# owl-project/owlExaBrick

Measured on AMD Instinct MI355X. Metric: frames/sec at 2048^2 DVR, exajet-like, MI355X, higher is better.
Workload: dtype f32; 1 GPU; c4_exajet (seed 0xe7a0003 procedural AMR, scale 1.0): 640512000 cells / 1251000 bricks / 13349488 regions, 2048x2048 DVR, dt 0.5, alpha ramp, gradient shading on, space skipping on, frameID 0; tiling=16x16 tiles interleaved over 1 GPU(s)

## Files before the change

### owlexabrick_amd/csrc/exa_kernels.hip

```cpp
#include "exa_device.h"
#include <cfloat>

#if EXA_BASIS_FORM == 0 && EXA_EMPTY_CELLS
#define EXA_FORM_NS form0e
#elif EXA_BASIS_FORM == 0
#define EXA_FORM_NS form0
#elif EXA_BASIS_FORM == 1 && EXA_EMPTY_CELLS
#error "empty cells are a per-corner property: the per-axis association (EXA_BASIS_FORM 1) does not apply"
#elif EXA_BASIS_FORM == 1
#define EXA_FORM_NS form1
#else
#error "EXA_BASIS_FORM is 0 (source order) or 1 (per-axis association with fused multiply-adds)"
#endif
#define EXA_F1 (EXA_BASIS_FORM == 1)
#ifndef EXA_TU_ROPE
#define EXA_TU_ROPE 0
#endif
#ifndef EXA_TU_SAMPLE
#define EXA_TU_SAMPLE 0
#endif
#ifndef EXA_TU_STREAM
#define EXA_TU_STREAM 0
#endif
namespace exa {
namespace EXA_FORM_NS {

struct V3 { float x, y, z; };
__device__ __forceinline__ V3 mk(float x, float y, float z) { V3 r; r.x = x; r.y = y; r.z = z; return r; }
__device__ __forceinline__ V3 mk(const float *p) { return mk(p[0], p[1], p[2]); }
__device__ __forceinline__ V3 operator+(V3 a, V3 b) { return mk(a.x + b.x, a.y + b.y, a.z + b.z); }
__device__ __forceinline__ V3 operator-(V3 a, V3 b) { return mk(a.x - b.x, a.y - b.y, a.z - b.z); }
__device__ __forceinline__ V3 operator*(float s, V3 a) { return mk(s * a.x, s * a.y, s * a.z); }
__device__ __forceinline__ V3 operator-(V3 a) { return mk(-a.x, -a.y, -a.z); }
__device__ __forceinline__ float dot(V3 a, V3 b) { return a.x * b.x + a.y * b.y + a.z * b.z; }
__device__ __forceinline__ float dotF(V3 a, V3 b) { return EXA_F1 ? __builtin_fmaf(a.z, b.z, __builtin_fmaf(a.y, b.y, a.x * b.x)) : dot(a, b); }
__device__ __forceinline__ V3 gradOf(float sumW, float sumWV, V3 sumD, V3 sumDC)
{
  return EXA_F1 ? mk(__builtin_fmaf(sumW, sumD.x, -(sumWV * sumDC.x)), __builtin_fmaf(sumW, sumD.y, -(sumWV * sumDC.y)),
                     __builtin_fmaf(sumW, sumD.z, -(sumWV * sumDC.z)))
                : mk(sumW * sumD.x - sumWV * sumDC.x, sumW * sumD.y - sumWV * sumDC.y, sumW * sumD.z - sumWV * sumDC.z);
}
__device__ __forceinline__ V3 rayAt(V3 org, float t, V3 dir)
{ return EXA_F1 ? mk(__builtin_fmaf(t, dir.x, org.x), __builtin_fmaf(t, dir.y, org.y), __builtin_fmaf(t, dir.z, org.z)) : org + t * dir; }
__device__ __forceinline__ float length(V3 a) { return sqrtf(dot(a, a)); }
__device__ __forceinline__ V3 normalize(V3 a) { return (1.f / sqrtf(dot(a, a))) * a; }
__device__ __forceinline__ V3 cross(V3 a, V3 b)
{ return mk(a.y * b.z - a.z * b.y, a.z * b.x - a.x * b.z, a.x * b.y - a.y * b.x); }

__device__ __forceinline__ V3 xfmPoint(const ExaHipFrameState &fs, V3 p)
{ return p.x * mk(fs.xfm_vx) + (p.y * mk(fs.xfm_vy) + (p.z * mk(fs.xfm_vz) + mk(fs.xfm_p))); }
__device__ __forceinline__ V3 xfmVector(const ExaHipFrameState &fs, V3 v)
{ return v.x * mk(fs.xfm_vx) + (v.y * mk(fs.xfm_vy) + v.z * mk(fs.xfm_vz)); }

struct Lcg {
  uint32_t state;
  __device__ __forceinline__ void init(uint32_t v0, uint32_t v1)
  {
    uint32_t s0 = 0;
#pragma unroll
    for (int n = 0; n < 16; n++) {
      s0 += 0x9e3779b9u;
      v0 += ((v1 << 4) + 0xa341316cu) ^ (v1 + s0) ^ ((v1 >> 5) + 0xc8013ea4u);
      v1 += ((v0 << 4) + 0xad90777du) ^ (v0 + s0) ^ ((v0 >> 5) + 0x7e95761eu);
    }
    state = v0;
  }
  __device__ __forceinline__ float next()
  {
    state = 1664525u * state + 1013904223u;
    return float(state & 0x00FFFFFFu) / float(0x01000000);
  }
};

template <bool FAST> __device__ __forceinline__ float fdiv(float a, float b) { return FAST ? a * __builtin_amdgcn_rcpf(b) : a / b; }
template <bool FAST> __device__ __forceinline__ float fdivExact(float a, float b, float y )
{
  if (!FAST) return a / b;
  const float q = __builtin_amdgcn_fmed3f(a * y, -3.402823466e+38f, 3.402823466e+38f);
  return __builtin_fmaf(__builtin_fmaf(-q, b, a), y, q);
}
template <bool FAST> __device__ __forceinline__ float fdivExact(float a, float b) { return fdivExact<FAST>(a, b, FAST ? __builtin_amdgcn_rcpf(b) : 0.f); }
template <bool FAST> __device__ __forceinline__ float fsqrt(float a) { return FAST ? __builtin_amdgcn_sqrtf(a) : sqrtf(a); }

struct Ray { V3 org, dir; float tmin, tmax; };
// ... 143 lines not shown
    if (ha && hb) {
      const bool aFirst = a0 <= b0;
      stack[sp * 256] = aFirst ? cc.y : cc.x;
      sp++;
      node = aFirst ? cc.x : cc.y;
    } else if (ha) {
      node = cc.x;
    } else if (hb) {
      node = cc.y;
    } else {
      if (sp == 0) break;
      sp--;
      node = stack[sp * 256];
    }
  }
  return best;
}

struct Basis { float sumWV, sumW; V3 sumD, sumDC; };

template <bool DERIV, int STATS>
__device__ __forceinline__ void addBasisFunctions(Ctx<STATS> &C, Basis &B, const int4 b0, const int4 b1,
                                                  const float *__restrict__ field, V3 pos)
{
  const int sx = b0.w, sy = b1.x, sz = b1.y;
  const float invCw = __int_as_float((127 - b1.z) << 23);
  const float lpx = (pos.x - float(b0.x)) * invCw - 0.5f;
  const float lpy = (pos.y - float(b0.y)) * invCw - 0.5f;
  const float lpz = (pos.z - float(b0.z)) * invCw - 0.5f;
  const int lx = max(-1, int(floorf(lpx))), ly = max(-1, int(floorf(lpy))), lz = max(-1, int(floorf(lpz)));
  const int hx = lx + 1, hy = ly + 1, hz = lz + 1;
  const float fx = lpx - float(lx), fy = lpy - float(ly), fz = lpz - float(lz);
  const float nx = 1.f - fx, ny = 1.f - fy, nz = 1.f - fz;
  const bool vlx = lx >= 0 && lx < sx, vhx = hx < sx;
  const bool vly = ly >= 0 && ly < sy, vhy = hy < sy;
  const bool vlz = lz >= 0 && lz < sz, vhz = hz < sz;
  const int cxl = min(max(lx, 0), sx - 1), cxh = min(hx, sx - 1);
  const int cyl = min(max(ly, 0), sy - 1), cyh = min(hy, sy - 1);
  const int czl = min(max(lz, 0), sz - 1), czh = min(hz, sz - 1);
  const uint32_t base = (uint32_t)b1.w;
  const uint32_t rowLL = base + (uint32_t)(cyl * sx + czl * sx * sy);
  const uint32_t rowHL = base + (uint32_t)(cyh * sx + czl * sx * sy);
  const uint32_t rowLH = base + (uint32_t)(cyl * sx + czh * sx * sy);
  const uint32_t rowHH = base + (uint32_t)(cyh * sx + czh * sx * sy);
  const float s000 = field[rowLL + cxl], s100 = field[rowLL + cxh];
  const float s010 = field[rowHL + cxl], s110 = field[rowHL + cxh];
  const float s001 = field[rowLH + cxl], s101 = field[rowLH + cxh];
  const float s011 = field[rowHH + cxl], s111 = field[rowHH + cxh];
  C.count(ST_BRICK_VISITS);
#define EXA_CORNER(VALID, S, WZ, WY, WX, SGX, SGY, SGZ)                                     \
  {                                                                                          \
     \
    const bool v_ = (VALID) && (!EXA_EMPTY_CELLS || (S) != EXA_EMPTY_CELL_POISON_VALUE);     \
    if (STATS == 1 && (VALID)) C.st[ST_CORNER_LOADS]++;                                      \
    const float w_ = (WZ) * (WY) * (WX);                                                     \
    if (DERIV) {                                                                             \
      const float dx_ = (WZ) * (WY) * (SGX 1.f);                                             \
      const float dy_ = (WZ) * (WX) * (SGY 1.f);                                             \
      const float dz_ = (WY) * (WX) * (SGZ 1.f);                                             \
      B.sumDC.x = v_ ? B.sumDC.x + dx_ : B.sumDC.x;                                          \
      B.sumDC.y = v_ ? B.sumDC.y + dy_ : B.sumDC.y;                                          \
      B.sumDC.z = v_ ? B.sumDC.z + dz_ : B.sumDC.z;                                          \
      B.sumD.x = v_ ? B.sumD.x + dx_ * (S) : B.sumD.x;                                       \
      B.sumD.y = v_ ? B.sumD.y + dy_ * (S) : B.sumD.y;                                       \
      B.sumD.z = v_ ? B.sumD.z + dz_ * (S) : B.sumD.z;                                       \
    }                                                                                        \
    B.sumW = v_ ? B.sumW + w_ : B.sumW;                                                      \
    B.sumWV = v_ ? B.sumWV + w_ * (S) : B.sumWV;                                             \
  }
  EXA_CORNER(vlz && vly && vlx, s000, nz, ny, nx, -, -, -)
  EXA_CORNER(vlz && vly && vhx, s100, nz, ny, fx, +, -, -)
  EXA_CORNER(vlz && vhy && vlx, s010, nz, fy, nx, -, +, -)
  EXA_CORNER(vlz && vhy && vhx, s110, nz, fy, fx, +, +, -)
  EXA_CORNER(vhz && vly && vlx, s001, fz, ny, nx, -, -, +)
  EXA_CORNER(vhz && vly && vhx, s101, fz, ny, fx, +, -, +)
  EXA_CORNER(vhz && vhy && vlx, s011, fz, fy, nx, -, +, +)
  EXA_CORNER(vhz && vhy && vhx, s111, fz, fy, fx, +, +, +)
#undef EXA_CORNER
}

struct __attribute__((packed, aligned(4))) Pair { float a, b; };
__device__ __forceinline__ Pair loadPair(const float *__restrict__ p) { return *reinterpret_cast<const Pair *>(p); }

template <bool DERIV, int STATS, bool SMALL, bool VOXEL = false, bool CUBE = false>
__device__ __forceinline__ void addBasisFast(Ctx<STATS> &C, Basis &B, const int4 b0, const int4 b1,
                                             const float *__restrict__ field, V3 pos, const int cubeLog2 = 0)
{
  static_assert(!CUBE || SMALL, "cube records: the 32-bit address form only");
  const int sx = CUBE ? (1 << cubeLog2) : b1.x, sy = CUBE ? sx : b1.y, sz = CUBE ? sx : b1.z;
  const uint32_t begin = CUBE ? ((uint32_t)b0.w >> 9) << (3 * cubeLog2) : (uint32_t)b1.w;
  const float invCw = __int_as_float(CUBE ? (int)((uint32_t)b0.w << 23) : b0.w);
  const float lpx = EXA_F1 ? __builtin_fmaf(pos.x - __int_as_float(b0.x), invCw, -0.5f) : (pos.x - __int_as_float(b0.x)) * invCw - 0.5f;
  const float lpy = EXA_F1 ? __builtin_fmaf(pos.y - __int_as_float(b0.y), invCw, -0.5f) : (pos.y - __int_as_float(b0.y)) * invCw - 0.5f;
  const float lpz = EXA_F1 ? __builtin_fmaf(pos.z - __int_as_float(b0.z), invCw, -0.5f) : (pos.z - __int_as_float(b0.z)) * invCw - 0.5f;
  const float flx = fmaxf(floorf(lpx), -1.f), fly = fmaxf(floorf(lpy), -1.f), flz = fmaxf(floorf(lpz), -1.f);
  const int lx = int(flx), ly = int(fly), lz = int(flz);
  const int hx = lx + 1, hy = ly + 1, hz = lz + 1;
  const float fx = lpx - flx, fy = lpy - fly, fz = lpz - flz;
  const bool vlx = (uint32_t)lx < (uint32_t)sx, vhx = hx < sx;
  const bool vly = (uint32_t)ly < (uint32_t)sy, vhy = hy < sy;
  const bool vlz = (uint32_t)lz < (uint32_t)sz, vhz = hz < sz;
  auto med3 = [](int a, int c) {
    int r;
    if (CUBE) asm("v_med3_i32 %0, %1, 0, %2" : "=v"(r) : "v"(a), "s"(c));
    else asm("v_med3_i32 %0, %1, 0, %2" : "=v"(r) : "v"(a), "v"(c));
    return r;
  };
  const int cxl = med3(lx, sx - 1), cxh = min(hx, sx - 1);
  const int cyl = med3(ly, sy - 1), cyh = min(hy, sy - 1);
  const int czl = med3(lz, sz - 1), czh = min(hz, sz - 1);
  const int bx = med3(lx, CUBE ? sx - 2 : max(sx - 2, 0));
  float s000, s100, s010, s110, s001, s101, s011, s111;
  {
    uint32_t rowLL, rowHL, rowLH, rowHH;
    if (CUBE) {
      const uint32_t at = begin + (uint32_t)bx;
      const uint32_t zl = ((uint32_t)czl << (2 * cubeLog2)) + at, zh = ((uint32_t)czh << (2 * cubeLog2)) + at;
      rowLL = ((uint32_t)cyl << cubeLog2) + zl; rowHL = ((uint32_t)cyh << cubeLog2) + zl;
      rowLH = ((uint32_t)cyl << cubeLog2) + zh; rowHH = ((uint32_t)cyh << cubeLog2) + zh;
    } else if (SMALL) {
      const uint32_t sxy = __umul24((uint32_t)sx, (uint32_t)sy);
      const uint32_t zl = __umul24((uint32_t)czl, sxy) + (begin + (uint32_t)bx);
      const uint32_t zh = __umul24((uint32_t)czh, sxy) + (begin + (uint32_t)bx);
      const uint32_t yl = __umul24((uint32_t)cyl, (uint32_t)sx), yh = __umul24((uint32_t)cyh, (uint32_t)sx);
      rowLL = zl + yl; rowHL = zl + yh; rowLH = zh + yl; rowHH = zh + yh;
    } else {
      const uint32_t sxy = (uint32_t)(sx * sy);
      const uint32_t zl = begin + (uint32_t)czl * sxy + (uint32_t)bx, zh = begin + (uint32_t)czh * sxy + (uint32_t)bx;
      const uint32_t yl = (uint32_t)(cyl * sx), yh = (uint32_t)(cyh * sx);
      rowLL = zl + yl; rowHL = zl + yh; rowLH = zh + yl; rowHH = zh + yh;
    }
    const bool lFirst = cxl == bx, hFirst = cxh == bx;
    Pair pLL, pHL, pLH, pHH;
    if (SMALL) {
      const char *base = reinterpret_cast<const char *>(field);
      pLL = *reinterpret_cast<const Pair *>(base + (rowLL << 2)); pHL = *reinterpret_cast<const Pair *>(base + (rowHL << 2));
      pLH = *reinterpret_cast<const Pair *>(base + (rowLH << 2)); pHH = *reinterpret_cast<const Pair *>(base + (rowHH << 2));
    } else {
      pLL = loadPair(field + rowLL); pHL = loadPair(field + rowHL);
      pLH = loadPair(field + rowLH); pHH = loadPair(field + rowHH);
    }
    s000 = lFirst ? pLL.a : pLL.b; s100 = hFirst ? pLL.a : pLL.b;
    s010 = lFirst ? pHL.a : pHL.b; s110 = hFirst ? pHL.a : pHL.b;
    s001 = lFirst ? pLH.a : pLH.b; s101 = hFirst ? pLH.a : pLH.b;
    s011 = lFirst ? pHH.a : pHH.b; s111 = hFirst ? pHH.a : pHH.b;
  }
  C.count(ST_BRICK_VISITS);
  if (STATS == 1) {
    const int nx = lpx != lpx ? (1 + int(1 < sx)) : (int(vlx) + int(vhx));
    const int ny = lpy != lpy ? (1 + int(1 < sy)) : (int(vly) + int(vhy));
    const int nz = lpz != lpz ? (1 + int(1 < sz)) : (int(vlz) + int(vhz));
    C.st[ST_CORNER_LOADS] += (unsigned)(nx * ny * nz);
  }
  const float wxl = vlx ? 1.f - fx : 0.f, wxh = vhx ? fx : 0.f;
  const float wyl = vly ? 1.f - fy : 0.f, wyh = vhy ? fy : 0.f;
  const float wzl = vlz ? 1.f - fz : 0.f, wzh = vhz ? fz : 0.f;
#if EXA_BASIS_FORM == 1
  {
    const float aLL = __builtin_fmaf(wxh, s100, wxl * s000), aLH = __builtin_fmaf(wxh, s110, wxl * s010);
    const float aHL = __builtin_fmaf(wxh, s101, wxl * s001), aHH = __builtin_fmaf(wxh, s111, wxl * s011);
    const float Al = __builtin_fmaf(wyh, aLH, wyl * aLL), Ah = __builtin_fmaf(wyh, aHH, wyl * aHL);
    B.sumWV = __builtin_fmaf(wzh, Ah, __builtin_fmaf(wzl, Al, B.sumWV));
    const float Sx = wxl + wxh, Sy = wyl + wyh, Sz = wzl + wzh;
    const float zy = Sz * Sy;
    B.sumW = __builtin_fmaf(zy, Sx, B.sumW);
    if (DERIV) {
      const float dw = VOXEL ? invCw : 1.f;
      const float mxl = vlx ? -dw : 0.f, mxh = vhx ? dw : 0.f;
      const float myl = vly ? -dw : 0.f, myh = vhy ? dw : 0.f;
      const float mzl = vlz ? -dw : 0.f, mzh = vhz ? dw : 0.f;
      const float dLL = __builtin_fmaf(mxh, s100, mxl * s000), dLH = __builtin_fmaf(mxh, s110, mxl * s010);
      const float dHL = __builtin_fmaf(mxh, s101, mxl * s001), dHH = __builtin_fmaf(mxh, s111, mxl * s011);
      const float DXl = __builtin_fmaf(wyh, dLH, wyl * dLL), DXh = __builtin_fmaf(wyh, dHH, wyl * dHL);
      const float DYl = __builtin_fmaf(myh, aLH, myl * aLL), DYh = __builtin_fmaf(myh, aHH, myl * aHL);
      B.sumD.x = __builtin_fmaf(wzh, DXh, __builtin_fmaf(wzl, DXl, B.sumD.x));
      B.sumD.y = __builtin_fmaf(wzh, DYh, __builtin_fmaf(wzl, DYl, B.sumD.y));
      B.sumD.z = __builtin_fmaf(mzh, Ah, __builtin_fmaf(mzl, Al, B.sumD.z));
      const float Mx = mxl + mxh, My = myl + myh, Mz = mzl + mzh;
      B.sumDC.x = __builtin_fmaf(zy, Mx, B.sumDC.x);
      B.sumDC.y = __builtin_fmaf(Sz * Sx, My, B.sumDC.y);
      B.sumDC.z = __builtin_fmaf(Sy * Sx, Mz, B.sumDC.z);
    }
  }
#else
  const float zyLL = wzl * wyl, zyLH = wzl * wyh, zyHL = wzh * wyl, zyHH = wzh * wyh;
  if (DERIV) {
    const float dw = VOXEL ? invCw : 1.f;
    const float mxl = vlx ? -dw : 0.f, mxh = vhx ? dw : 0.f;
    const float myl = vly ? -dw : 0.f, myh = vhy ? dw : 0.f;
    const float mzl = vlz ? -dw : 0.f, mzh = vhz ? dw : 0.f;
    const float zxLL = wzl * wxl, zxLH = wzl * wxh, zxHL = wzh * wxl, zxHH = wzh * wxh;
    const float yxLL = wyl * wxl, yxLH = wyl * wxh, yxHL = wyh * wxl, yxHH = wyh * wxh;
#define EXA_ACC(S, ZY0, WX, MX, ZX0, MY, YX0, MZ)                                            \
    {                                                                                        \
      const bool ne_ = !EXA_EMPTY_CELLS || (S) != EXA_EMPTY_CELL_POISON_VALUE;               \
      const float ZY = ne_ ? (ZY0) : 0.f, ZX = ne_ ? (ZX0) : 0.f, YX = ne_ ? (YX0) : 0.f;    \
      B.sumDC.x = __builtin_fmaf((ZY), (MX), B.sumDC.x);                                     \
      B.sumDC.y = __builtin_fmaf((ZX), (MY), B.sumDC.y);                                     \
      B.sumDC.z = __builtin_fmaf((YX), (MZ), B.sumDC.z);                                     \
      B.sumD.x = __builtin_fmaf((ZY) * (S), (MX), B.sumD.x);                                 \
      B.sumD.y = __builtin_fmaf((ZX) * (S), (MY), B.sumD.y);                                 \
      B.sumD.z = __builtin_fmaf((YX) * (S), (MZ), B.sumD.z);                                 \
      const float w_ = (ZY) * (WX);                                                          \
      B.sumW += w_; B.sumWV += w_ * (S);                                                     \
    }
    EXA_ACC(s000, zyLL, wxl, mxl, zxLL, myl, yxLL, mzl)
    EXA_ACC(s100, zyLL, wxh, mxh, zxLH, myl, yxLH, mzl)
    EXA_ACC(s010, zyLH, wxl, mxl, zxLL, myh, yxHL, mzl)
    EXA_ACC(s110, zyLH, wxh, mxh, zxLH, myh, yxHH, mzl)
    EXA_ACC(s001, zyHL, wxl, mxl, zxHL, myl, yxLL, mzh)
    EXA_ACC(s101, zyHL, wxh, mxh, zxHH, myl, yxLH, mzh)
    EXA_ACC(s011, zyHH, wxl, mxl, zxHL, myh, yxHL, mzh)
    EXA_ACC(s111, zyHH, wxh, mxh, zxHH, myh, yxHH, mzh)
#undef EXA_ACC
  } else {
#define EXA_ACC(S, ZY, WX) { const float w_ = (!EXA_EMPTY_CELLS || (S) != EXA_EMPTY_CELL_POISON_VALUE) ? (ZY) * (WX) : 0.f; B.sumW += w_; B.sumWV += w_ * (S); }
    EXA_ACC(s000, zyLL, wxl) EXA_ACC(s100, zyLL, wxh) EXA_ACC(s010, zyLH, wxl) EXA_ACC(s110, zyLH, wxh)
    EXA_ACC(s001, zyHL, wxl) EXA_ACC(s101, zyHL, wxh) EXA_ACC(s011, zyHH, wxl) EXA_ACC(s111, zyHH, wxh)
#undef EXA_ACC
  }
#endif
}

template <int NCH> struct __attribute__((packed, aligned(4))) PairN { float v[2 * NCH]; };
// ... 1454 lines not shown
}
__global__ __launch_bounds__(256) void aoFinalizeKernel(const RenderArgs a)
{
  const unsigned numHits = a.aoCount[0];
  for (unsigned h = blockIdx.x * 256u + threadIdx.x; h < numHits; h += gridDim.x * 256u) {
    const AoRecord *r = a.aoRecs + h;
    const float4 posFd = r->posFd, ngAmb = r->ngAmb, baseRnd = r->baseRnd;
    const uint32_t slot = r->slot;
    const int hitCnt = (int)a.aoHit[2u * h] + (int)a.aoHit[2u * h + 1u];
    const float shadow = (float)hitCnt / 2;
    const float fd = posFd.w;
    const float ns = 1.f - shadow;
    const float t_hit = a.surf[slot].w;
    a.surf[slot] = make_float4(ngAmb.w + baseRnd.x * fd * ns, ngAmb.w + baseRnd.y * fd * ns, ngAmb.w + baseRnd.z * fd * ns, t_hit);
  }
}

#endif

template <bool ISO_ONLY, bool SORTED>
__global__ __launch_bounds__(kKdBlock, (ISO_ONLY ? EXA_AO_ISO_WAVES : EXA_PREPASS_WAVES)) void aoRaysKdKernel(const RenderArgs a)
{
  static_assert(ldsFits(kdLds(1), ISO_ONLY ? EXA_AO_ISO_WAVES : EXA_PREPASS_WAVES), "LDS per workgroup x waves per SIMD exceeds the CU's 160 KB");
  const LdsPtrs lds = carveLds(kdLds(a.numXfChannels));
  Ctx<0> C;
  kernelPrologue(C, a, lds);
  float *stackF = lds.stackF, *qT = lds.qT;
  int *qRegion = lds.qRegion;
  C.fastSampler = a.fastSampler != 0;
  const ExaHipFrameState &fs = a.fs;
  const unsigned numRays = 2u * a.aoCount[0];
  for (;;) {
    unsigned base = 0;
    if ((threadIdx.x & 63) == 0) base = atomicAdd(&a.aoCount[2], 64u);
    base = (unsigned)__shfl((int)base, 0, 64);
    if (base >= numRays) break;
    const unsigned k = base + (threadIdx.x & 63);
    const bool live = k < numRays;
    const unsigned j = (SORTED && live) ? a.aoOrder[k] : k;
    int hitFlag = 0;
    float4 posFd = make_float4(0.f, 0.f, 0.f, 0.f), ngAmb = posFd, baseRnd = posFd;
    uint32_t slot = 0;
    if (live) {
      const AoRecord *r = a.aoRecs + (j >> 1);
      posFd = r->posFd; ngAmb = r->ngAmb; baseRnd = r->baseRnd; slot = r->slot;
      const Ray ao_ray = aoRayOf(fs, posFd, ngAmb, baseRnd, j);
      SurfaceHit ao;
      traceSurfacesKd<0, ISO_ONLY>(C, ao_ray, ao, false, stackF, qRegion, qT);
      if (ao.primID >= 0 || ao.primID == EXA_PRIMID_ISOSURFACE || ao.primID == EXA_PRIMID_PLANE
          || ao.primID == EXA_PRIMID_STREAMLINE) hitFlag = 1;
      if (SORTED) a.aoHit[j] = (uint8_t)hitFlag;
    }
    if (SORTED) continue;
    const int other = __shfl_xor(hitFlag, 1, 64);
    if (live && !(j & 1u)) {
      const int hitCnt = hitFlag + other;
      const float shadow = (float)hitCnt / 2;
      const float fd = posFd.w;
      const float ns = 1.f - shadow;
      const float t_hit = a.surf[slot].w;
      a.surf[slot] = make_float4(ngAmb.w + baseRnd.x * fd * ns, ngAmb.w + baseRnd.y * fd * ns, ngAmb.w + baseRnd.z * fd * ns, t_hit);
    }
  }
  if (C.guardTripped) atomicExch(a.errorFlag, 1);
}

constexpr int marchWaves(int MULTI, int STATS, bool SMALL, int NCH, bool ROPE)
{
  return NCH > 1 ? (NCH == 2 ? EXA_IL2_WAVES : EXA_IL34_WAVES)
             : (MULTI == 1 ? EXA_MULTI_WAVES
                           : (MULTI ? 5 : ((ROPE && !STATS && SMALL && EXA_BASIS_FORM == 1) ? EXA_ROPE_WAVES : EXA_MARCH_WAVES)));
}

template <bool GRAD, bool FAST, int MULTI, bool SURF, int STATS, bool SMALL, int NCH = 0, bool ROPE = false>
__global__ __launch_bounds__(kKdBlock, marchWaves(MULTI, STATS, SMALL, NCH, ROPE)) void renderFrameKdKernel(const RenderArgs a)
{
  constexpr bool CUBE = NCH == 1;
  constexpr int IL = CUBE ? 0 : NCH;
  static_assert(!CUBE || (MULTI == 0 && ROPE && SMALL && STATS == 0 && EXA_BASIS_FORM == 1 && !EXA_EMPTY_CELLS),
                "the cube records are a variant of the shipped one-channel 32-bit rope march");
#ifndef EXA_CUBE_LEAN
#define EXA_CUBE_LEAN 0
#endif
  constexpr bool LEAN = marchWaves(MULTI, STATS, SMALL, NCH, ROPE) >= 7 && (!CUBE || EXA_CUBE_LEAN);
  constexpr int PACKED_CT = !ROPE ? -1 : (STATS == 1 ? 0 : (SMALL ? 1 : -1));
  const bool packedRec = PACKED_CT < 0 ? a.leafBeginBits != 0 : PACKED_CT != 0;
  static_assert(IL == 0 || (MULTI == 2 && STATS == 0), "the interleaved march is a multi-channel variant of the shipped kernel");
  constexpr int KS = marchLds(MULTI == 1, false, 0).stackEntries;
  constexpr int QN = marchLds(MULTI == 1, ROPE, 0).queueEntries;
  static_assert(ldsFits(marchLds(MULTI == 1, ROPE, IL ? IL : (MULTI ? 2 : 1)), marchWaves(MULTI, STATS, SMALL, NCH, ROPE)),
                "LDS per workgroup x waves per SIMD exceeds the CU's 160 KB: shorten the queue or lower the occupancy");
  const LdsPtrs lds = carveLds(marchLds(MULTI == 1, ROPE, a.numXfChannels));
  float4 *queue4 = lds.queue4;
  float *stackF = lds.stackF, *qT = lds.qT;
  int *qRegion = lds.qRegion;
  for (int i = threadIdx.x; i < a.numXfChannels * EXA_NUM_XF_VALUES; i += kKdBlock) lds.xf[i] = a.xf[i];
  __syncthreads();
  Ctx<STATS> C;
  initCtx(C, a, lds);
  const unsigned long long clockBegin = clock64();
  if (STATS) for (int i = 0; i < ST_COUNT; i++) C.st[i] = 0;
  __shared__ unsigned long long lapMarks[STATS == 2 ? 8 * (kKdBlock / 64) : 1];
  if (STATS == 2) {
    C.lapMark = lapMarks + 8 * (threadIdx.x >> 6);
    if ((threadIdx.x & 63) == 0) {
      C.lapMark[0] = clock64(); C.lapMark[1] = ST_T_OTHER - ST_T_BRICK;
      for (int i = 2; i < 7; i++) C.lapMark[i] = 0;
    }
  }

  const int wavesPerBlock = kKdBlock / 64;
  const int gwave = blockIdx.x * wavesPerBlock + (threadIdx.x >> 6);
  const int tile = a.tileMap[gwave >> 2];
  const int tx = tile % a.tilesX, ty = tile / a.tilesX;
  const int wave = gwave & 3, lane = threadIdx.x & 63;
  const int inX = ((wave & 1) << 3) + laneX(lane), inY = ((wave >> 1) << 3) + laneY(lane);
  const int px = tx * kTile + inX, py = ty * kTile + inY;
  const bool inside = px < a.W && py < a.H && (a.debugPixel < 0 || a.debugPixel == px + a.W * py);

  if (STATS == 1 && a.walkProbe) C.probe = a.walkProbe + size_t(gwave) * kWalkProbeSize;
  unsigned marchIters = 0;
  if (inside) {
    const ExaHipFrameState &fs = a.fs;
    const int frameID = fs.frameID;
    Lcg rnd;
    Ray ray = cameraRay(a, px, py, rnd);
    float surface_t_hit = ray.tmax;
    if (SURF) {
      const size_t slot0 = slotOf(a, tile, inX, inY, px, py);
      surface_t_hit = a.surf[slot0].w;
      rnd.state = a.surfRnd[slot0];
    }
    const float interleavedSamplingOffset = rnd.next();
    clipToVoxelSpace(fs, ray, surface_t_hit);
    ray.org.x = __int_as_float(__builtin_amdgcn_readfirstlane(__float_as_int(ray.org.x)));
    ray.org.y = __int_as_float(__builtin_amdgcn_readfirstlane(__float_as_int(ray.org.y)));
    ray.org.z = __int_as_float(__builtin_amdgcn_readfirstlane(__float_as_int(ray.org.z)));

    Color4 pixelColor; pixelColor.x = pixelColor.y = pixelColor.z = pixelColor.w = 0.f;
    const int numChannels = a.p.numPrimaryChannels;

    KdWalk w;
    w.pk.v = 0;
    {
      Ray whole = ray; whole.tmin = -INFINITY; whole.tmax = INFINITY;
      float r0, r1;
      const bool hit = boxTest(whole, mk(a.kdLo), mk(a.kdHi), r0, r1);
      w.tn = fmaxf(r0, ray.tmin);
      w.tf = fminf(r1, ray.tmax);
      w.tEnd = w.tf;
      w.ref = (hit && w.tn < w.tf) ? (ROPE ? a.ropeRoot : a.kdMarchRoot) : EXA_KD_DONE;
    }
    bool ropeFast = false;
    if (ROPE) ropeFast = a.ropeFastDiv != 0 && !anyLane(!ropeRayInRange(ray));

    float walkTmin = ray.tmin;

    bool haveSeg = false;
    int listBegin = 0, listSize = 0;
    float flcw = 1.f;
    float t1 = 0.f, t_i = 0.f, t_sample = 0.f, actual_dt = 0.f;
    int child = 0, chan = 0;
    int4 hb0 = make_int4(0, 0, 0, 1), hb1 = make_int4(1, 1, 1, 0);
    Basis B;
    B.sumWV = 0.f; B.sumW = 0.f; B.sumD = mk(0.f, 0.f, 0.f); B.sumDC = mk(0.f, 0.f, 0.f);
    float xWV[IL > 1 ? IL - 1 : 1];
    V3 xD[IL > 1 ? IL - 1 : 1];
#pragma unroll
    for (int c = 0; c < (IL > 1 ? IL - 1 : 1); c++) { xWV[c] = 0.f; xD[c] = mk(0.f, 0.f, 0.f); }
    const float *field0 = a.sc.scalars + a.sc.channelOffset[0];
    const float *field = field0;
    float xfRcpRange0 = 0.f, xfRange0 = 0.f;
    if (FAST && !MULTI) {
      xfRange0 = __int_as_float(__builtin_amdgcn_readfirstlane(__float_as_int((fs.xfDomain[0][1] - fs.xfDomain[0][0]) + 1e-20f)));
      xfRcpRange0 = __int_as_float(__builtin_amdgcn_readfirstlane(__float_as_int(__builtin_amdgcn_rcpf(xfRange0))));
    }
    float xfRcpRangeN[IL ? IL : 1], xfRangeN[IL ? IL : 1];
#pragma unroll
    for (int c = 0; c < (IL ? IL : 1); c++) {
      xfRangeN[c] = (FAST && IL) ? __int_as_float(__builtin_amdgcn_readfirstlane(__float_as_int((fs.xfDomain[c][1] - fs.xfDomain[c][0]) + 1e-20f))) : 0.f;
      xfRcpRangeN[c] = (FAST && IL) ? __int_as_float(__builtin_amdgcn_readfirstlane(__float_as_int(__builtin_amdgcn_rcpf(xfRangeN[c])))) : 0.f;
    }

    unsigned iter = 0;
    for (;; iter++) {
      if (iter == 0xfffffff0u) { C.guardTripped = true; break; }
      if (anyLane(!haveSeg && w.pk.get(PK_QCOUNT) == 0 && w.ref != EXA_KD_DONE)) {
        C.lap(ST_T_WALK);
        do {
          const bool want = w.pk.get(PK_QCOUNT) < QN && w.ref != EXA_KD_DONE;
          if (want) {
            if (ROPE) ropeStep<STATS, SMALL, QN, LEAN, PACKED_CT>(C, w, walkTmin, a, queue4, ray, ropeFast, interleavedSamplingOffset);
            else kdStep<false, STATS, SMALL, KS>(C, w, walkTmin, a, stackF, qRegion, qT, ray, 0, walkTmin, 1.f, a.kdMarchNodes, a.kdMarchRoot);
          }
        } while (anyLane(!haveSeg && w.pk.get(PK_QCOUNT) == 0 && w.ref != EXA_KD_DONE));
      }
      if (!haveSeg) {
        C.lap(ST_T_SEG);
        const int qc = w.pk.get(PK_QCOUNT);
        if (qc == 0) break;
        const int qh = w.pk.get(PK_QHEAD);
        int region;
        float t0, tiQueued = 0.f;
        if (ROPE) {
          const float4 e = queue4[qh * kKdBlock];
          region = __float_as_int(e.x); t1 = e.y; tiQueued = e.z; t0 = e.w;
        } else {
          region = qRegion[qh * kKdBlock];
          t0 = qT[(2 * qh) * kKdBlock];
          t1 = qT[(2 * qh + 1) * kKdBlock];
        }
        w.pk.template incWrap<QN>(PK_QHEAD);
        w.pk.dec(PK_QCOUNT);
        if (packedRec) {
          const unsigned d = (unsigned)region;
          listBegin = (int)(d & ((1u << a.leafBeginBits) - 1u));
          listSize = (int)((d >> a.leafBeginBits) & ((1u << a.leafSizeBits) - 1u)) + 1;
          flcw = __int_as_float((127 + (int)(d >> (a.leafBeginBits + a.leafSizeBits))) << 23);
        } else {
          const RegionInfo ri = a.sc.regionInfo[region];
          listBegin = ri.listBegin; listSize = ri.listSize;
          flcw = ri.finestLevelCellWidth;
        }
        C.count(ST_SEGMENTS);
        haveSeg = true;
        w.pk.setBit(PK_NEEDHDR);
        if (ROPE && packedRec)
          t_i = tiQueued;
        else if (a.invDtPow2 != 0.f)
          t_i = firstSampleTPow2(t0, a.p.dt * flcw, a.invDtPow2 * __int_as_float(0x7f000000 - __float_as_int(flcw)), interleavedSamplingOffset);
        else
          t_i = firstSampleT(t0, a.p.dt * flcw, interleavedSamplingOffset);
        {
          const float t_next = fminf(t_i, t1);
          t_sample = 0.5f * (fminf(t1, t_next) + t0);
          actual_dt = t_next - t0;
        }
        C.count(ST_SAMPLE_EVALS);
      }

      C.lap(ST_T_BRICK);
      C.phase(ST_W_BRICK);
      if (listSize > 1 || w.pk.get(PK_NEEDHDR)) {
        if (CUBE) {
          hb0 = *reinterpret_cast<const int4 *>(reinterpret_cast<const char *>(a.leafHdrCube) + ((uint32_t)(listBegin + child) << 4));
        } else if (SMALL) {
          const char *hp = reinterpret_cast<const char *>(a.sc.leafHdr) + ((uint32_t)(listBegin + child) << 5);
          hb0 = *reinterpret_cast<const int4 *>(hp); hb1 = *reinterpret_cast<const int4 *>(hp + 16);
        } else {
          const unsigned at = 2u * (unsigned)(listBegin + child);
          hb0 = a.sc.leafHdr[at]; hb1 = a.sc.leafHdr[at + 1u];
        }
        w.pk.clearField(PK_NEEDHDR);
      }
      if (IL) addBasisFastIl<GRAD, SMALL, (IL ? IL : 2)>(B, xWV, xD, hb0, hb1, a.cellsIl, rayAt(ray.org, t_sample, ray.dir));
      else if (CUBE) addBasisFast<GRAD, STATS, SMALL, false, CUBE>(C, B, hb0, hb1, field0, rayAt(ray.org, t_sample, ray.dir), a.cubeLog2);
      else addBasisFast<GRAD, STATS, SMALL>(C, B, hb0, hb1, MULTI ? field : field0, rayAt(ray.org, t_sample, ray.dir));
      child++;
      if (child < listSize) continue;

      C.lap(ST_T_FINAL);
      C.phase(ST_W_FINAL);
      if (IL) {
        if (B.sumW > 1e-20f) {
#pragma unroll
          for (int c = 0; c < IL; c++) {
            const float wv = c == 0 ? B.sumWV : xWV[c == 0 ? 0 : c - 1];
            const V3 sd = c == 0 ? B.sumD : xD[c == 0 ? 0 : c - 1];
            const float cellValue = fdivExact<FAST>(wv, B.sumW);
            V3 grad = mk(0.f, 0.f, 0.f);
            if (GRAD) grad = gradOf(B.sumW, wv, sd, B.sumDC);
            integrateVolume<FAST, STATS, FAST>(C, ray, pixelColor, actual_dt, cellValue, grad, flcw, c, xfRcpRangeN[c], xfRangeN[c]);
          }
        }
#pragma unroll
        for (int c = 0; c < (IL > 1 ? IL - 1 : 1); c++) { xWV[c] = 0.f; xD[c] = mk(0.f, 0.f, 0.f); }
      } else if (B.sumW > 1e-20f) {
        C.count(ST_SAMPLES);
        const float cellValue = fdivExact<FAST>(B.sumWV, B.sumW);
        V3 grad = mk(0.f, 0.f, 0.f);
        if (GRAD) grad = gradOf(B.sumW, B.sumWV, B.sumD, B.sumDC);
        integrateVolume<FAST, STATS, (FAST && !MULTI), LEAN>(C, ray, pixelColor, actual_dt, cellValue, grad, flcw, MULTI ? chan : 0, xfRcpRange0, xfRange0);
      }
      B.sumWV = 0.f; B.sumW = 0.f; B.sumD = mk(0.f, 0.f, 0.f); B.sumDC = mk(0.f, 0.f, 0.f);
      child = 0;
      if (MULTI && !IL) {
        chan++;
        if (chan < numChannels) {
          field = a.sc.scalars + a.sc.channelOffset[chan];
          C.count(ST_SAMPLE_EVALS);
          continue;
        }
        chan = 0; field = field0;
      }
      if (pixelColor.w >= EXA_TERMINATION_THRESHOLD) {
        pixelColor.x = pixelColor.x * pixelColor.w;
        pixelColor.y = pixelColor.y * pixelColor.w;
        pixelColor.z = pixelColor.z * pixelColor.w;
        pixelColor.w = 1.f;
        break;
      }
      const float t_last = fminf(t_i, t1);
      if (t_last >= t1) {
        haveSeg = false;
        continue;
      }
      t_i += a.p.dt * flcw;
      {
        const float t_next = fminf(t_i, t1);
        t_sample = 0.5f * (fminf(t1, t_next) + t_last);
        actual_dt = t_next - t_last;
      }
      C.count(ST_SAMPLE_EVALS);
    }

    C.lap(ST_T_OTHER);
    marchIters = iter;
    size_t slot, colorSlot;
    {
      unsigned tid = threadIdx.x, bid = blockIdx.x;
      asm volatile("" : "+v"(tid));
      asm volatile("" : "+s"(bid));
      const int lane2 = tid & 63, wave2 = (tid >> 6) & 3;
      const int inX2 = ((wave2 & 1) << 3) + laneX(lane2), inY2 = ((wave2 >> 1) << 3) + laneY(lane2);
      slot = (a.world == 1) ? size_t(tx * kTile + inX2) + size_t(a.W) * (ty * kTile + inY2)
                            : size_t(a.tileMap[(bid * wavesPerBlock + (tid >> 6)) >> 2] / a.world) * kTilePixels + (inY2 * kTile + inX2);
      colorSlot = a.colorRowMajor ? size_t(tx * kTile + inX2) + size_t(a.W) * (ty * kTile + inY2) : slot;
    }
    if (SURF && a.pixOut) {
      a.pixOut[slot] = make_float4(pixelColor.x, pixelColor.y, pixelColor.z, pixelColor.w);
    } else {
    float4 bgColor = make_float4(0.f, 0.f, 0.f, 0.f);
    if (SURF) bgColor = a.surf[slot];
    float cr = pixelColor.w * pixelColor.x + (1.f - pixelColor.w) * bgColor.x;
    float cg = pixelColor.w * pixelColor.y + (1.f - pixelColor.w) * bgColor.y;
    float cb = pixelColor.w * pixelColor.z + (1.f - pixelColor.w) * bgColor.z;
    if (fs.clockScale > 0.f) cr = clockHeat(fs.clockScale, clockBegin);
    if (frameID > 0) {
      const float4 acc = a.accum[slot];
      cr += acc.x; cg += acc.y; cb += acc.z;
    }
    a.accum[slot] = make_float4(cr, cg, cb, 1.f);
    const float div = frameID + 1.f;
    cr = cr / div; cg = cg / div; cb = cb / div;
    a.color[colorSlot] = make_rgba8(linear_to_srgb(cr), linear_to_srgb(cg), linear_to_srgb(cb));
    }
  }

  if (a.tileCost) {
    unsigned v = marchIters;
    for (int off = 32; off > 0; off >>= 1) v = max(v, (unsigned)__shfl_down((int)v, off, 64));
    unsigned bid = blockIdx.x, tid = threadIdx.x;
    asm volatile("" : "+s"(bid));
    asm volatile("" : "+v"(tid));
    if (lane == 0) atomicMax(&a.tileCost[a.tileMap[(bid * wavesPerBlock + (tid >> 6)) >> 2]], v);
  }
  if (C.guardTripped) atomicExch(a.errorFlag, 1);
  if (STATS == 2) {
    if (lane < 5 && C.lapMark[2 + lane]) atomicAdd(&a.stats[ST_T_BRICK + lane], C.lapMark[2 + lane]);
  }
  if (STATS == 1) {
    for (int i = 0; i < ST_COUNT; i++) {
      unsigned long long v = inside ? C.st[i] : 0ull;
      for (int off = 32; off > 0; off >>= 1) v += __shfl_down(v, off, 64);
      if ((threadIdx.x & 63) == 0 && v) atomicAdd(&a.stats[i], v);
    }
    __shared__ unsigned wgMaxIters;
    if (threadIdx.x == 0) wgMaxIters = 0;
    __syncthreads();
    unsigned v = marchIters;
    for (int off = 32; off > 0; off >>= 1) v = max(v, (unsigned)__shfl_down((int)v, off, 64));
    if (lane == 0) atomicMax(&wgMaxIters, v);
    __syncthreads();
    if (lane == 0) atomicAdd(&a.stats[ST_WAVE_ITERS], (unsigned long long)v);
    if (threadIdx.x == 0) atomicAdd(&a.stats[ST_TILE_ITERS], 4ull * wgMaxIters);
  }
}

__device__ __forceinline__ void kdCollectStep(Ctx<0> &C, KdWalk &w, const float winLo, const float winHi, const RenderArgs &a,
                                              float *stackF, const Ray &ray, const KdNodeDev *nodes, const int root,
                                              float4 *out, unsigned &count)
{
  if (w.ref != EXA_KD_EMPTY && !(w.tn < winHi)) { w.ref = EXA_KD_DONE; return; }
  if (w.ref < 0 && w.ref > EXA_KD_DONE) {
    if (w.tn >= winLo && w.tn < w.tf) out[count++] = make_float4(__int_as_float(~w.ref), w.tn, w.tf, 0.f);
    w.ref = EXA_KD_EMPTY;
  }
  if (w.ref == EXA_KD_EMPTY || (w.ref != EXA_KD_DONE && !(w.tf > winLo))) kdPop(C, w, root, stackF, nodes, ray);
  if (w.ref < 0 || !(w.tf > winLo) || !(w.tn < winHi)) return;
  kdNodeStage<kKdStackEntries, false, 0>(C, w, stackF, ray, nodes, 2);
}

template <bool GRAD, bool FAST, bool SURF, int L, bool SMALL>
__global__ __launch_bounds__(kKdBlock, 4) void renderFrameKdWideKernel(const RenderArgs a)
{
  static_assert(ldsFits(kdLds(1), 4), "LDS per workgroup x waves per SIMD exceeds the CU's 160 KB");
  const LdsPtrs lds = carveLds(kdLds(a.numXfChannels));
  float *stackF = lds.stackF;
// ... 696 lines not shown
```

Measured before the change: 63.90 frames/s.

## Defer sample shading until the next sample's field loads are in flight

In the cube-record march, shading and compositing of the previous sample are deferred and executed between the issue of the next sample's corner loads and their use. This hides the global-memory latency of the trilinear fetch behind the transfer-function and gradient work. It also turns on the LEAN integrate path when deferring with gradients. The risk is extra live registers (pending state, basis sums kept across iterations), which can lower occupancy, plus wasted loads issued for a sample past early termination.

```diff
diff --git a/owlexabrick_amd/csrc/exa_kernels.hip b/owlexabrick_amd/csrc/exa_kernels.hip
--- a/owlexabrick_amd/csrc/exa_kernels.hip
+++ b/owlexabrick_amd/csrc/exa_kernels.hip
@@ -1,5 +1,6 @@
 #include "exa_device.h"
 #include <cfloat>
+#include <type_traits>
 
 #if EXA_BASIS_FORM == 0 && EXA_EMPTY_CELLS
 #define EXA_FORM_NS form0e
@@ -309,9 +310,10 @@
 struct __attribute__((packed, aligned(4))) Pair { float a, b; };
 __device__ __forceinline__ Pair loadPair(const float *__restrict__ p) { return *reinterpret_cast<const Pair *>(p); }
 
-template <bool DERIV, int STATS, bool SMALL, bool VOXEL = false, bool CUBE = false>
+struct NothingBetween { __device__ __forceinline__ bool operator()() const { return true; } };
+template <bool DERIV, int STATS, bool SMALL, bool VOXEL = false, bool CUBE = false, class Between = NothingBetween>
 __device__ __forceinline__ void addBasisFast(Ctx<STATS> &C, Basis &B, const int4 b0, const int4 b1,
-                                             const float *__restrict__ field, V3 pos, const int cubeLog2 = 0)
+                                             const float *__restrict__ field, V3 pos, const int cubeLog2 = 0, Between between = Between())
 {
   static_assert(!CUBE || SMALL, "cube records: the 32-bit address form only");
   const int sx = CUBE ? (1 << cubeLog2) : b1.x, sy = CUBE ? sx : b1.y, sz = CUBE ? sx : b1.z;
@@ -367,6 +369,7 @@
       pLL = loadPair(field + rowLL); pHL = loadPair(field + rowHL);
       pLH = loadPair(field + rowLH); pHH = loadPair(field + rowHH);
     }
+    if constexpr (!std::is_same<Between, NothingBetween>::value) { if (!between()) return; }
     s000 = lFirst ? pLL.a : pLL.b; s100 = hFirst ? pLL.a : pLL.b;
     s010 = lFirst ? pHL.a : pHL.b; s110 = hFirst ? pHL.a : pHL.b;
     s001 = lFirst ? pLH.a : pLH.b; s101 = hFirst ? pLH.a : pLH.b;
@@ -1987,7 +1990,11 @@
 #ifndef EXA_CUBE_LEAN
 #define EXA_CUBE_LEAN 0
 #endif
-  constexpr bool LEAN = marchWaves(MULTI, STATS, SMALL, NCH, ROPE) >= 7 && (!CUBE || EXA_CUBE_LEAN);
+#ifndef EXA_MARCH_DEFER
+#define EXA_MARCH_DEFER 1
+#endif
+  constexpr bool DEFER = CUBE && EXA_MARCH_DEFER;
+  constexpr bool LEAN = marchWaves(MULTI, STATS, SMALL, NCH, ROPE) >= 7 && (!CUBE || EXA_CUBE_LEAN || (DEFER && GRAD));
   constexpr int PACKED_CT = !ROPE ? -1 : (STATS == 1 ? 0 : (SMALL ? 1 : -1));
   const bool packedRec = PACKED_CT < 0 ? a.leafBeginBits != 0 : PACKED_CT != 0;
   static_assert(IL == 0 || (MULTI == 2 && STATS == 0), "the interleaved march is a multi-channel variant of the shipped kernel");
@@ -2086,6 +2093,19 @@
       xfRangeN[c] = (FAST && IL) ? __int_as_float(__builtin_amdgcn_readfirstlane(__float_as_int((fs.xfDomain[c][1] - fs.xfDomain[c][0]) + 1e-20f))) : 0.f;
       xfRcpRangeN[c] = (FAST && IL) ? __int_as_float(__builtin_amdgcn_readfirstlane(__float_as_int(__builtin_amdgcn_rcpf(xfRangeN[c])))) : 0.f;
     }
+
+    bool pending = false;
+    float pendDt = 0.f, pendFlcw = 1.f;
+    auto shadePending = [&]() {
+      if (B.sumW > 1e-20f) {
+        const float cellValue = fdivExact<FAST>(B.sumWV, B.sumW);
+        V3 grad = mk(0.f, 0.f, 0.f);
+        if (GRAD) grad = gradOf(B.sumW, B.sumWV, B.sumD, B.sumDC);
+        integrateVolume<FAST, STATS, (FAST && !MULTI), LEAN>(C, ray, pixelColor, pendDt, cellValue, grad, pendFlcw, 0, xfRcpRange0, xfRange0);
+      }
+      B.sumWV = 0.f; B.sumW = 0.f; B.sumD = mk(0.f, 0.f, 0.f); B.sumDC = mk(0.f, 0.f, 0.f);
+      pending = false;
+    };
 
     unsigned iter = 0;
     for (;; iter++) {
@@ -2158,6 +2178,39 @@
         }
         w.pk.clearField(PK_NEEDHDR);
       }
+      if (DEFER) {
+        bool ended = false;
+        addBasisFast<GRAD, STATS, SMALL, false, CUBE>(C, B, hb0, hb1, field0, rayAt(ray.org, t_sample, ray.dir), a.cubeLog2, [&]() {
+          if (pending) {
+            shadePending();
+            ended = pixelColor.w >= EXA_TERMINATION_THRESHOLD;
+          }
+          return !ended;
+        });
+        if (ended) {
+          pixelColor.x = pixelColor.x * pixelColor.w;
+          pixelColor.y = pixelColor.y * pixelColor.w;
+          pixelColor.z = pixelColor.z * pixelColor.w;
+          pixelColor.w = 1.f;
+          break;
+        }
+        child++;
+        if (child < listSize) continue;
+        child = 0;
+        pending = true; pendDt = actual_dt; pendFlcw = flcw;
+        const float t_last = fminf(t_i, t1);
+        if (t_last >= t1) {
+          haveSeg = false;
+          continue;
+        }
+        t_i += a.p.dt * flcw;
+        {
+          const float t_next = fminf(t_i, t1);
+          t_sample = 0.5f * (fminf(t1, t_next) + t_last);
+          actual_dt = t_next - t_last;
+        }
+        continue;
+      }
       if (IL) addBasisFastIl<GRAD, SMALL, (IL ? IL : 2)>(B, xWV, xD, hb0, hb1, a.cellsIl, rayAt(ray.org, t_sample, ray.dir));
       else if (CUBE) addBasisFast<GRAD, STATS, SMALL, false, CUBE>(C, B, hb0, hb1, field0, rayAt(ray.org, t_sample, ray.dir), a.cubeLog2);
       else addBasisFast<GRAD, STATS, SMALL>(C, B, hb0, hb1, MULTI ? field : field0, rayAt(ray.org, t_sample, ray.dir));
@@ -2219,6 +2272,15 @@
       C.count(ST_SAMPLE_EVALS);
     }
 
+    if (DEFER && pending) {
+      shadePending();
+      if (pixelColor.w >= EXA_TERMINATION_THRESHOLD) {
+        pixelColor.x = pixelColor.x * pixelColor.w;
+        pixelColor.y = pixelColor.y * pixelColor.w;
+        pixelColor.z = pixelColor.z * pixelColor.w;
+        pixelColor.w = 1.f;
+      }
+    }
     C.lap(ST_T_OTHER);
     marchIters = iter;
     size_t slot, colorSlot;
```

New measurement: 66.04 frames/s, median of 6. +3.4%, better.
